# tachyon-beep/shogidrl

Measured on NVIDIA B200. Metric: legal-masked Shogi env steps/sec, higher is better.
Workload: dtype u8

## Files before the change

### shogidrl_b200/csrc/kz_engine.cu

```cuda
#include <cuda_runtime.h>
#include <stddef.h>
#include <stdint.h>
#include "../../include/keisei_b200.h"
#include "kz_common.cuh"

namespace {

__device__ uint32_t g_ray[81 * 8 * 3];
__device__ uint32_t g_step[NCLS * 81 * 3];
__device__ uint32_t g_init_bitmap[BITMAP_WORDS];

__constant__ uint8_t c_init_board[96];
__constant__ uint32_t c_init_key_w;

struct __align__(16) WarpScratch {
  uint32_t bitmap[BITMAP_WORDS];
  uint8_t board[96];
  uint8_t meta[32];
  uint8_t pind[2][96];
  uint32_t pinl[2][8 * 3];
  uint8_t plist[2][40];
  uint8_t dropv[96];
  uint32_t oimg[72];
  float opv[20];
  uint32_t onz;
  uint32_t pad_[3];
};

__shared__ uint32_t s_ray[81 * 8 * 3];
__shared__ uint32_t s_step[NCLS * 81 * 3];
extern __shared__ __align__(16) unsigned char s_dyn[];
#define s_ws (reinterpret_cast<WarpScratch*>(s_dyn))

struct Tables {};

#ifndef KZ_FILL_UNROLL
#define KZ_FILL_UNROLL 1
#endif
#ifndef KZ_FILL_AFTER_COMPACT
#define KZ_FILL_AFTER_COMPACT 1
#endif
#ifndef KZ_ST256
#define KZ_ST256 3
#endif
#ifndef KZ_ROWS_ONCE
#define KZ_ROWS_ONCE 1
#endif
#ifndef KZ_BULK_ZERO
#define KZ_BULK_ZERO 0
#endif
constexpr int kFillUnroll = KZ_FILL_UNROLL;

#if KZ_BULK_ZERO
constexpr int kZeroPage = 16384;
__shared__ __align__(128) unsigned char s_zero[kZeroPage];
__device__ __forceinline__ void bulk_zero(void* dst, uint32_t bytes) {
  const uint32_t src = (uint32_t)__cvta_generic_to_shared(s_zero);
  asm volatile("cp.async.bulk.global.shared::cta.bulk_group [%0], [%1], %2;" ::"l"(dst), "r"(src), "r"(bytes) : "memory");
}
#endif

__device__ __forceinline__ void st_zero256(void* p) {
  const uint32_t z = 0;
  asm volatile("st.global.v8.b32 [%0], {%1,%1,%1,%1,%1,%1,%1,%1};" ::"l"(p), "r"(z) : "memory");
}

__device__ __forceinline__ void st256(void* p, const uint32_t (&v)[8]) {
  asm volatile("st.global.v8.b32 [%0], {%1,%2,%3,%4,%5,%6,%7,%8};" ::"l"(p), "r"(v[0]), "r"(v[1]), "r"(v[2]), "r"(v[3]),
               "r"(v[4]), "r"(v[5]), "r"(v[6]), "r"(v[7]) : "memory");
}

__device__ __forceinline__ BB ld_ray(const Tables&, int sq, int d) {
  const uint32_t* p = s_ray + (sq * 8 + d) * 3;
  return BB{p[0], p[1], p[2]};
}
__device__ __forceinline__ BB ld_step(const Tables&, int cls, int sq) {
  const uint32_t* p = s_step + (cls * 81 + sq) * 3;
  return BB{p[0], p[1], p[2]};
}

__device__ __forceinline__ BB slide_ray(const Tables& T, int sq, int d, BB occ) {
  BB ray = ld_ray(T, sq, d);
  BB bl = ray & occ;
  if (bb_any(bl)) {
    if (dir_positive(d)) ray = ray & bb_upto(bb_lsb(bl));
    else ray = bb_andn(ray, bb_below(bb_msb(bl)));
  }
  return ray;
}

#ifndef KD_ATTR
#define KD_ATTR __forceinline__
#endif
__device__ KD_ATTR BB king_danger(const uint32_t tab, const int K, const int me, const BB occk) {
  const int lane = threadIdx.x & 31;
  const WarpScratch& ws = s_ws[threadIdx.x >> 5];
  const Tables T{};
  const int fwd = me == 0 ? -1 : 1;
  const BB kingsteps = ld_step(T, CLS_KING, K);
// ... 376 lines not shown
  k.z = fmix32(id * 0xC2B2AE3Du + 0x27D4EB2Fu);
  k.w = fmix32(id * 0x27D4EB2Fu + 0x9E3779B9u);
  return k;
}
__device__ __forceinline__ uint4 position_key(const WarpScratch& ws, int lane, int side) {
  uint4 k = make_uint4(0, 0, 0, 0);
#pragma unroll
  for (int j = 0; j < 3; j++) {
    const int sq = lane + 32 * j;
    const int code = sq < 81 ? ws.board[sq] : 0;
    if (code) { uint4 t = zkey_item(sq * 32 + code); k.x ^= t.x; k.y ^= t.y; k.z ^= t.z; k.w ^= t.w; }
  }
  if (lane < 14) {
    const int cnt = ws.meta[lane];
    if (cnt) { uint4 t = zkey_item(4096 + lane * 256 + cnt); k.x ^= t.x; k.y ^= t.y; k.z ^= t.z; k.w ^= t.w; }
  }
  if (lane == 31 && side) { uint4 t = zkey_item(8191); k.x ^= t.x; k.y ^= t.y; k.z ^= t.z; k.w ^= t.w; }
  k.x = __reduce_xor_sync(FULL, k.x);
  k.y = __reduce_xor_sync(FULL, k.y);
  k.z = __reduce_xor_sync(FULL, k.z);
  k.w = __reduce_xor_sync(FULL, k.w);
  return k;
}

struct StepParams {
  uint8_t* boards;
  uint8_t* meta;
  uint4* hist;
  int rep_slots;
  int hist_cap;
  int n;
  int g_first;
  const void* actions;
  int actions_i64;
  float* obs;
  long long obs_stride;
  uint8_t* mask;
  long long mask_stride;
  int mask_vec;
  float* reward;
  uint8_t* done;
  uint8_t* reason;
  int8_t* winner;
  int32_t* ep_len;
  int32_t* legal_count;
  uint8_t* in_check;
  void* next_actions;
  unsigned long long seed;
  uint32_t rng_step;
  uint32_t env_offset;
  int auto_reset;
  int mode;
  int eval_term;
  int* tile_counter;
  uint32_t* bitmap_out;
  long long bitmap_stride;
  uint32_t* cobs_out;
  const uint32_t* pool;
  int pool_size;
  const int32_t* pool_pick;
  unsigned long long pool_seed;
  int32_t* start_ids;
};

__device__ __forceinline__ uint16_t ld_u16(const uint8_t* p) { return (uint16_t)(p[0] | (p[1] << 8)); }
__device__ __forceinline__ void st_u16(uint8_t* p, int v) { p[0] = (uint8_t)v; p[1] = (uint8_t)(v >> 8); }

template <int MODE, bool POOL = false>
__global__ void __launch_bounds__(WARPS_PER_CTA * 32, MIN_CTAS_PER_SM) kz_step_kernel(const StepParams P) {
  for (int i = threadIdx.x; i < 81 * 8 * 3; i += blockDim.x) s_ray[i] = g_ray[i];
  for (int i = threadIdx.x; i < NCLS * 81 * 3; i += blockDim.x) s_step[i] = g_step[i];
#if KZ_BULK_ZERO
  for (int i = threadIdx.x; i < kZeroPage / 16; i += blockDim.x) reinterpret_cast<uint4*>(s_zero)[i] = make_uint4(0, 0, 0, 0);
  asm volatile("fence.proxy.async.shared::cta;" ::: "memory");
#endif
  __syncthreads();
  const Tables T{};
  const int lane = threadIdx.x & 31, warp = threadIdx.x >> 5;
  WarpScratch& ws = s_ws[warp];
  const uint32_t tab = code_info(lane);
  const int g_end = P.g_first + P.n;

  auto fetch_state = [&](int g) -> uint32_t {
    if (g >= g_end) return 0u;
    const uint8_t* src = lane < 24 ? P.boards + (size_t)g * 96 + 4 * lane : P.meta + (size_t)g * 32 + 4 * (lane - 24);
    return *reinterpret_cast<const uint32_t*>(src);
  };
  auto fetch_action = [&](int g) -> long long {
    if (g >= g_end || MODE == 0) return 0;
    return P.actions_i64 ? reinterpret_cast<const long long*>(P.actions)[g]
                         : (long long)reinterpret_cast<const int*>(P.actions)[g];
  };
  const bool lockstep = (P.n % WARPS_PER_CTA) == 0 && P.tile_counter != nullptr;
  const int ntiles = P.n / WARPS_PER_CTA;
  __shared__ int s_tile[4];
  int tile = blockIdx.x, pending = 0;
  if (lockstep && threadIdx.x == 0) {
    s_tile[1] = gridDim.x + atomicAdd(P.tile_counter, 1);
    pending = gridDim.x + atomicAdd(P.tile_counter, 1);
  }
  const int g_stride = gridDim.x * WARPS_PER_CTA;
  int g = P.g_first + blockIdx.x * WARPS_PER_CTA + warp;
  uint32_t next_word = fetch_state(g);
  long long next_action = fetch_action(g);
  __syncthreads();

  for (int it = 0; lockstep ? tile < ntiles : g < g_end; it++) {
    int g_next = g + g_stride;
    if (lockstep) {
      __syncthreads();
      tile = s_tile[(it + 1) & 3];
      g_next = P.g_first + tile * WARPS_PER_CTA + warp;
      if (threadIdx.x == 0) s_tile[(it + 2) & 3] = pending;
    }
    __syncwarp();
    static_assert(offsetof(WarpScratch, meta) == offsetof(WarpScratch, board) + 96, "meta must follow board: one store for all 32 lanes");
    reinterpret_cast<uint32_t*>(ws.board)[lane] = next_word;
    const long long a = next_action;
    next_word = fetch_state(g_next);
    next_action = fetch_action(g_next);
    __syncwarp();
    int side = ws.meta[14];
    int status = ws.meta[15];
    int winner = ws.meta[16] == 0xFF ? -1 : ws.meta[16];
    int err = ws.meta[17];
    int move_count = ld_u16(ws.meta + 18);
    int hist_len = ld_u16(ws.meta + 20);
    const int max_moves = ld_u16(ws.meta + 22);
    uint32_t episodes = ws.meta[24] | (ws.meta[25] << 8) | (ws.meta[26] << 16) | (ws.meta[27] << 24);



    float reward = 0.f;
    int done_out = 0, reason_out = 0, winner_out = -1, ep_len_out = 0;
    bool fresh_senn = false;
    int mover = 1 - side;
    bool moved = false;
    uint4 key = make_uint4(reinterpret_cast<const uint32_t*>(ws.board)[21], reinterpret_cast<const uint32_t*>(ws.board)[22],
                           reinterpret_cast<const uint32_t*>(ws.board)[23], reinterpret_cast<const uint32_t*>(ws.meta)[7]);
    uint32_t kid = 0;
    bool probe = false;
    uint4 probe_e = make_uint4(0, 0, 0, 0);

    if (MODE != 0) {
      if (status != 0) {
      } else if (a < 0 || a >= KZ_NUM_ACTIONS) {
        err |= KZ_ERR_BAD_ACTION;
      } else {
        mover = side;
        const int ai = (int)a;
        bool ok = true;
        if (ai < 12960) {
          const int promo = ai & 1, pair = ai >> 1;
          const int from = pair / 80, t80 = pair - from * 80, to = t80 + (t80 >= from);
          const int code = ws.board[from], tcode = ws.board[to];
          const uint32_t inf = __shfl_sync(FULL, tab, code);
          if (!code || code_color(code) != side) { err |= KZ_ERR_BAD_ACTION; ok = false; }
          else {
            const int fr = sq_row(from), fc = from - 9 * fr, tr = sq_row(to), tc = to - 9 * tr;
            const int dr = tr - fr, dc = tc - fc;
            bool pat;
            if (code_type(code) == 2) {
              pat = dr == (side == 0 ? -2 : 2) && (dc == 1 || dc == -1);
            } else {
              int d = -1;
              if (dc == 0) d = dr < 0 ? 0 : 4;
// ... 68 lines not shown
            key.w ^= __reduce_xor_sync(FULL, dk.w);
          }
          if (hist_len < P.hist_cap) {
            probe = true;
            probe_e = (P.hist + (size_t)g * P.rep_slots)[(key.y + lane) & ((uint32_t)P.rep_slots - 1u)];
            hist_len += 1;
          } else {
            err |= KZ_ERR_HISTORY_FULL;
          }
        }
      }
    }

    auto fill_mask_zero = [&]() {
      if (!P.mask || !P.mask_vec) return;
      uint8_t* mrow = P.mask + (size_t)g * P.mask_stride;
#if (KZ_ST256 & 1)
      if ((((uintptr_t)mrow) & 31) == 0) {
#pragma unroll kFillUnroll
        for (int q = lane; q < 405; q += 32) st_zero256(mrow + 32 * q);
        return;
      }
#endif
      uint4* m4 = reinterpret_cast<uint4*>(mrow);
      const uint4 z4 = make_uint4(0, 0, 0, 0);
#pragma unroll kFillUnroll
      for (int q = lane; q < 810; q += 32) m4[q] = z4;
    };
    auto fill_obs_zero = [&]() {
      if (!P.obs) return;
      float* orow = P.obs + (size_t)g * P.obs_stride;
#if (KZ_ST256 & 2)
      float2* o2 = reinterpret_cast<float2*>(orow);
      const int head = (int)(((32u - (unsigned)((uintptr_t)orow & 31)) & 31u) >> 3);
      const int nb = (KZ_OBS_FLOATS * 4 - head * 8) >> 5;
      char* body = reinterpret_cast<char*>(orow) + head * 8;
      if (lane < head) o2[lane] = make_float2(0.f, 0.f);
#pragma unroll kFillUnroll
      for (int q = lane; q < nb; q += 32) st_zero256(body + 32 * q);
      const int tail0 = head + 4 * nb;
      if (lane < KZ_OBS_FLOATS / 2 - tail0) o2[tail0 + lane] = make_float2(0.f, 0.f);
#else
      const int mis = ((uintptr_t)orow & 15) ? 2 : 0;
      float4* o4 = reinterpret_cast<float4*>(orow + mis);
      const float4 zf = make_float4(0.f, 0.f, 0.f, 0.f);
#pragma unroll kFillUnroll
      for (int q = lane; q < 931; q += 32) o4[q] = zf;
      if (lane == 0) {
        float2* o2 = reinterpret_cast<float2*>(orow + (mis ? 0 : 3724));
        *o2 = make_float2(0.f, 0.f);
      }
#endif
    };
    auto build_obs_image = [&]() {
      __syncwarp();
      ws.oimg[lane] = 0; ws.oimg[lane + 32] = 0;
      if (lane < 8) ws.oimg[lane + 64] = 0;
      float pv = 0.f;
      if (lane < 14) {
        const int cnt = ws.meta[lane < 7 ? side * 7 + lane : (1 - side) * 7 + (lane - 7)];
        if (cnt > 0) pv = __fdiv_rn((float)cnt, 18.0f);
      } else if (lane == 14) pv = side == 0 ? 1.f : 0.f;
      else if (lane == 15) pv = max_moves > 0 ? __fdiv_rn((float)move_count, (float)max_moves) : 0.f;
      if (lane < 20) ws.opv[lane] = pv;
      const uint32_t nz = __ballot_sync(FULL, pv != 0.f);
      if (lane == 0) ws.onz = nz;
      __syncwarp();
#pragma unroll
      for (int j = 0; j < 3; j++) {
        const int sq = lane + 32 * j;
        const int code = sq < 81 ? ws.board[sq] : 0;
        if (code) {
          const int t = code_type(code), mine = code_color(code) == side;
          const int plane = t < 8 ? (mine ? 0 : 14) + t : (mine ? 8 : 22) + (t - 8);
          const int f = plane * 81 + (side == 0 ? sq : 80 - sq);
          atomicOr(&ws.oimg[f >> 5], 1u << (f & 31));
        }
      }
      __syncwarp();
    };
    auto write_obs = [&]() {
      if (!P.obs) return;
      float* orow = P.obs + (size_t)g * P.obs_stride;
#if (KZ_ROWS_ONCE & 2)
      {
        build_obs_image();
        float2* o2 = reinterpret_cast<float2*>(orow);
        const int head = (int)(((32u - (unsigned)((uintptr_t)orow & 31)) & 31u) >> 3);
        const int nb = (KZ_OBS_FLOATS * 4 - head * 8) >> 5;
        char* body = reinterpret_cast<char*>(orow) + head * 8;
        if (lane < head) {
          const uint32_t b2 = ws.oimg[0] >> (2 * lane);
          o2[lane] = make_float2((b2 & 1) ? 1.0f : 0.f, (b2 & 2) ? 1.0f : 0.f);
        }
#pragma unroll 1
        for (int q = lane; q < nb; q += 32) {
          const int r0 = 2 * head + 8 * q;
          char* dst = body + 32 * q;
          if (r0 + 8 <= 28 * 81) {
            const uint32_t bits = __funnelshift_r(ws.oimg[r0 >> 5], ws.oimg[(r0 >> 5) + 1], r0 & 31) & 0xFFu;
            if (bits == 0) st_zero256(dst);
            else {
              uint32_t v[8];
#pragma unroll
              for (int k = 0; k < 8; k++) v[k] = ((bits >> k) & 1) ? 0x3F800000u : 0u;
              st256(dst, v);
            }
          } else {
            const int x = r0 - 28 * 81;
            const int pl0 = x >= 0 ? (x * 1619) >> 17 : -1;
            const int nb0 = (pl0 + 1) * 81 - x;
            const uint32_t a = pl0 >= 0 ? __float_as_uint(ws.opv[pl0]) : 0u, b = __float_as_uint(ws.opv[pl0 + 1]);
            uint32_t bits = 0;
            if (pl0 < 0) bits = __funnelshift_r(ws.oimg[r0 >> 5], ws.oimg[(r0 >> 5) + 1], r0 & 31) & ((1u << nb0) - 1u);
            if (a == 0 && bits == 0 && (nb0 >= 8 || b == 0)) st_zero256(dst);
            else {
              uint32_t v[8];
#pragma unroll
              for (int k = 0; k < 8; k++) v[k] = k < nb0 ? (pl0 >= 0 ? a : (((bits >> k) & 1) ? 0x3F800000u : 0u)) : b;
              st256(dst, v);
            }
          }
        }
        const int tail0 = head + 4 * nb;
        if (lane < KZ_OBS_FLOATS / 2 - tail0) o2[tail0 + lane] = make_float2(0.f, 0.f);
        return;
      }
#endif
      float pv = 0.f;
      if (lane < 14) {
        const int cnt = ws.meta[lane < 7 ? side * 7 + lane : (1 - side) * 7 + (lane - 7)];
        if (cnt > 0) pv = __fdiv_rn((float)cnt, 18.0f);
      } else if (lane == 14) pv = side == 0 ? 1.f : 0.f;
      else if (lane == 15) pv = max_moves > 0 ? __fdiv_rn((float)move_count, (float)max_moves) : 0.f;
      fill_obs_zero();
      __syncwarp();
      uint32_t nzp = __ballot_sync(FULL, pv != 0.f);
      while (nzp) {
        const int i = __ffs(nzp) - 1;
        nzp &= nzp - 1;
        const float v = __shfl_sync(FULL, pv, i);
        float* pl = orow + (28 + i) * 81;
        pl[lane] = v;
        pl[lane + 32] = v;
        if (lane < 17) pl[lane + 64] = v;
      }
#pragma unroll
      for (int j = 0; j < 3; j++) {
        const int sq = lane + 32 * j;
        const int code = sq < 81 ? ws.board[sq] : 0;
        if (code) {
          const int t = code_type(code), mine = code_color(code) == side;
          const int plane = t < 8 ? (mine ? 0 : 14) + t : (mine ? 8 : 22) + (t - 8);
          orow[plane * 81 + (side == 0 ? sq : 80 - sq)] = 1.0f;
        }
      }
    };
    if (MODE == 0) key = position_key(ws, lane, side);
    GenResult gr;
    if constexpr (MODE != 0) {
      gr = gen_moves_impl<true, UFZ_FAST>(tab, side, UFZ_FAST);
    } else {
      int mode = UFZ_GENERIC;
      if (ws.meta[side * 7] > 0) {
        GenResult opp = gen_moves<false>(tab, 1 - side, UFZ_SKIP);
        if (opp.in_check) mode = UFZ_ALL;
      }
      gr = gen_moves<true>(tab, side, mode);
    }

    if (probe) {
      uint4* tb = P.hist + (size_t)g * P.rep_slots;
      const uint32_t smask = (uint32_t)P.rep_slots - 1u;
      uint32_t start = key.y & smask;
      int count = 0;
      uint4 e = probe_e;
      for (int round = 0; round * 32 < P.rep_slots; round++) {
        const uint32_t slot = (start + lane) & smask;
        if (round > 0) e = tb[slot];
        const bool occupied = (e.w & 15u) != 0;
        const bool match = occupied && e.x == key.x && e.y == key.y && e.z == key.z && ((e.w ^ key.w) >> 4) == 0;
        const uint32_t stop = __ballot_sync(FULL, match || !occupied);
        if (stop) {
          const int f = __ffs(stop) - 1;
          const uint32_t oldw = __shfl_sync(FULL, e.w, f);
          const bool was_match = (__ballot_sync(FULL, match) >> f) & 1;
          count = was_match ? min(15, (int)(oldw & 15u) + 1) : 1;
// ... 167 lines not shown
            const uint32_t parts[2] = {v.x, v.y};
            for (int b = 0; b < 7; b++) mrow[13520 + b] = (uint8_t)(parts[b >> 2] >> (8 * (b & 3)));
          }
        }
      } else {
        for (int i = lane; i < KZ_NUM_ACTIONS; i += 32) mrow[i] = (uint8_t)((ws.bitmap[i >> 5] >> (i & 31)) & 1);
      }
    };
    auto pick_next = [&]() {
      if (!P.next_actions) return;
      long long pick = -1;
      if (gr.count > 0) {
        const uint32_t r = rand32(P.seed, (unsigned long long)P.env_offset + (unsigned long long)g, P.rng_step);
        const int k = (int)(((unsigned long long)r * (unsigned long long)gr.count) >> 32);
        const int w0 = lane * 14;
        int pcs[14];
        int mycnt = 0;
#pragma unroll
        for (int i = 0; i < 14; i++) { pcs[i] = __popc(ws.bitmap[w0 + i]); mycnt += pcs[i]; }
        int incl = mycnt;
#pragma unroll
        for (int o = 1; o < 32; o <<= 1) { const int t = __shfl_up_sync(FULL, incl, o); if (lane >= o) incl += t; }
        const int excl = incl - mycnt;
        int found = -1;
        if (k >= excl && k < incl) {
          int rem = k - excl, widx = 0;
          bool open_ = true;
#pragma unroll
          for (int i = 0; i < 14; i++) {
            if (open_) {
              if (rem < pcs[i]) { widx = i; open_ = false; }
              else rem -= pcs[i];
            }
          }
          uint32_t wv = ws.bitmap[w0 + widx];
          for (int r = rem; r > 0; r--) wv &= wv - 1;
          found = (w0 + widx) * 32 + __ffs(wv) - 1;
        }
        const uint32_t who = __ballot_sync(FULL, found >= 0);
        pick = __shfl_sync(FULL, found, __ffs(who) - 1);
      }
      if (lane == 0) {
        if (P.actions_i64) reinterpret_cast<long long*>(P.next_actions)[g] = pick;
        else reinterpret_cast<int*>(P.next_actions)[g] = (int)pick;
      }
    };
    if (MODE == 2 || P.bitmap_out) {
      __syncwarp();
      uint4* dst = reinterpret_cast<uint4*>(P.bitmap_out + (size_t)g * P.bitmap_stride);
      for (int i = lane; i < BITMAP_WORDS / 4; i += 32) dst[i] = reinterpret_cast<const uint4*>(ws.bitmap)[i];
    }
    if constexpr (MODE != 2) write_mask();
    pick_next();
    write_obs();
    if (P.cobs_out) {
      __syncwarp();
      uint8_t* cb = reinterpret_cast<uint8_t*>(ws.oimg);
      if (lane < 21) ws.oimg[lane] = 0xFFFFFFFFu;
      float pv = 0.f;
      if (lane < 14) {
        const int cnt = ws.meta[lane < 7 ? side * 7 + lane : (1 - side) * 7 + (lane - 7)];
        if (cnt > 0) pv = __fdiv_rn((float)cnt, 18.0f);
      } else if (lane == 14) pv = side == 0 ? 1.f : 0.f;
      else if (lane == 15) pv = max_moves > 0 ? __fdiv_rn((float)move_count, (float)max_moves) : 0.f;
      if (lane < 19) ws.oimg[21 + lane] = lane < 18 ? __float_as_uint(pv) : 0u;
      __syncwarp();
#pragma unroll
      for (int j = 0; j < 3; j++) {
        const int sq = lane + 32 * j;
        const int code = sq < 81 ? ws.board[sq] : 0;
        if (code) {
          const int t = code_type(code), mine = code_color(code) == side;
          cb[side == 0 ? sq : 80 - sq] = (uint8_t)(t < 8 ? (mine ? 0 : 14) + t : (mine ? 8 : 22) + (t - 8));
        }
      }
      __syncwarp();
      uint32_t* dst = P.cobs_out + (size_t)g * KZ_COBS_WORDS;
      for (int i = lane; i < KZ_COBS_WORDS; i += 32) dst[i] = ws.oimg[i];
      __syncwarp();
    }

    __syncwarp();
    if (lane == 0) {
      ws.meta[14] = (uint8_t)side;
      ws.meta[15] = (uint8_t)status;
      ws.meta[16] = (uint8_t)(winner < 0 ? 0xFF : winner);
      ws.meta[17] = (uint8_t)err;
      st_u16(ws.meta + 18, move_count);
      st_u16(ws.meta + 20, hist_len);
      ws.meta[24] = (uint8_t)episodes; ws.meta[25] = (uint8_t)(episodes >> 8);
      ws.meta[26] = (uint8_t)(episodes >> 16); ws.meta[27] = (uint8_t)(episodes >> 24);
      reinterpret_cast<uint32_t*>(ws.board)[21] = key.x;
      reinterpret_cast<uint32_t*>(ws.board)[22] = key.y;
      reinterpret_cast<uint32_t*>(ws.board)[23] = key.z;
      reinterpret_cast<uint32_t*>(ws.meta)[7] = key.w;
    }
    __syncwarp();
    {
      uint32_t* bdst = reinterpret_cast<uint32_t*>(P.boards + (size_t)g * 96);
      uint32_t* mdst = reinterpret_cast<uint32_t*>(P.meta + (size_t)g * 32);
      if (lane < 24) bdst[lane] = reinterpret_cast<uint32_t*>(ws.board)[lane];
      else mdst[lane - 24] = reinterpret_cast<uint32_t*>(ws.meta)[lane - 24];
    }
    __syncwarp();
    if (lockstep && threadIdx.x == 0) pending = gridDim.x + atomicAdd(P.tile_counter, 1);
    g = g_next;
  }
#if KZ_BULK_ZERO
  asm volatile("cp.async.bulk.commit_group;" ::: "memory");
  asm volatile("cp.async.bulk.wait_group 0;" ::: "memory");
#endif
}

#ifndef KZ_EXPAND_CTAS_PER_SM
#define KZ_EXPAND_CTAS_PER_SM 1
#endif
#ifndef KZ_EXPAND_PRELOAD
#define KZ_EXPAND_PRELOAD 0
#endif
#ifndef KZ_EXPAND_SPARSE
#define KZ_EXPAND_SPARSE 0
#endif
#ifndef KZ_COMPACT_CTAS_PER_SM
#define KZ_COMPACT_CTAS_PER_SM 2
#endif
__global__ void __launch_bounds__(256) kz_expand_kernel(const uint8_t* __restrict__ boards, const uint8_t* __restrict__ meta,
                                                        const uint32_t* __restrict__ bitmap, int n, float* obs,
                                                        long long obs_stride, uint8_t* mask, long long mask_stride,
                                                        int mask_vec) {
  const int lane = threadIdx.x & 31, warp = threadIdx.x >> 5;
  auto expand = [](uint32_t b16) {
    uint4 v;
    v.x = ((b16 & 0xF) * 0x00204081u) & 0x01010101u;
    v.y = (((b16 >> 4) & 0xF) * 0x00204081u) & 0x01010101u;
    v.z = (((b16 >> 8) & 0xF) * 0x00204081u) & 0x01010101u;
    v.w = (((b16 >> 12) & 0xF) * 0x00204081u) & 0x01010101u;
    return v;
  };
  for (int g = blockIdx.x * 8 + warp; g < n; g += gridDim.x * 8) {
    const uint32_t* bm = bitmap + (size_t)g * BITMAP_WORDS;
    if (mask) {
      uint8_t* mrow = mask + (size_t)g * mask_stride;
      if (mask_vec) {
        uint4* m4 = reinterpret_cast<uint4*>(mrow);
#if KZ_EXPAND_SPARSE
        if (mask_stride >= 13536 && (((uintptr_t)mrow) & 31) == 0) {
          uint32_t wreg[27];
#pragma unroll
          for (int k = 0; k < 27; k++) wreg[k] = lane + 32 * k < 846 ? __ldg(bm + ((lane + 32 * k) >> 1)) : 0u;
#pragma unroll 1
          for (int q = lane; q < 423; q += 32) st_zero256(mrow + 32 * q);
          __syncwarp();
#pragma unroll
          for (int k = 0; k < 27; k++) {
            const int q = lane + 32 * k;
            const uint32_t half = (q & 1) ? (wreg[k] >> 16) : (wreg[k] & 0xFFFF);
            if (q < 846 && half) m4[q] = expand(half);
          }
        } else
#endif
        {
#if KZ_EXPAND_PRELOAD
        uint32_t wreg[27];
#pragma unroll
// ... 221 lines not shown
  if (g >= n) return;
  const Tables T{};
  const uint8_t* b = boards + (size_t)g * 96;
  const int sq = squares[g];
  const uint32_t tab = code_info(lane);
  const int code = (sq >= 0 && sq < 81) ? b[sq] : 0;
  const uint32_t inf = __shfl_sync(FULL, tab, code);
  const int me = code_color(code);
  uint32_t o[3], w[3];
#pragma unroll
  for (int j = 0; j < 3; j++) {
    const int s = lane + 32 * j;
    const int c = s < 81 ? b[s] : 0;
    o[j] = __ballot_sync(FULL, c != 0);
    w[j] = __ballot_sync(FULL, c != 0 && code_color(c) == me);
  }
  BB t = BB{0, 0, 0};
  if (code) {
    t = ld_step(T, (inf >> 16) & 15, sq);
    uint32_t sl = (inf >> 8) & 0xFF;
    while (sl) { const int d = __ffs(sl) - 1; sl &= sl - 1; t = t | slide_ray(T, sq, d, BB{o[0], o[1], o[2]}); }
    t = bb_andn(t, BB{w[0], w[1], w[2]});
  }
  if (lane == 0) { out[(size_t)g * 3] = t.w0; out[(size_t)g * 3 + 1] = t.w1; out[(size_t)g * 3 + 2] = t.w2; }
}

thread_local char t_cuda_err[256] = "";
int cuda_fail(cudaError_t e) {
  snprintf(t_cuda_err, sizeof t_cuda_err, "%s", cudaGetErrorString(e));
  return KZ_E_CUDA;
}
}
int kz_cuda_fail(cudaError_t e) { return cuda_fail(e); }
namespace {
#define CK(x) do { cudaError_t _e = (x); if (_e != cudaSuccess) return cuda_fail(_e); } while (0)

constexpr int kMaxDevices = 64;
int g_sm_counts[kMaxDevices] = {0};
bool g_ready[kMaxDevices] = {false};
inline int cur_device() { int d = 0; return cudaGetDevice(&d) == cudaSuccess && d >= 0 && d < kMaxDevices ? d : -1; }
inline bool host_ready() { const int d = cur_device(); return d >= 0 && g_ready[d]; }
inline int sm_count() { const int d = cur_device(); return d >= 0 ? g_sm_counts[d] : 0; }

struct Layout { int64_t off_boards, off_meta, off_hist, off_sched, total; int rep_slots; };
Layout layout(int n, int hist_cap) {
  Layout L;
  L.rep_slots = 64;
  while (L.rep_slots < 2 * hist_cap) L.rep_slots *= 2;
  L.off_boards = 0;
  L.off_meta = (int64_t)n * 96;
  L.off_hist = L.off_meta + (int64_t)n * 32;
  L.off_hist = (L.off_hist + 255) & ~(int64_t)255;
  L.off_sched = L.off_hist + (int64_t)n * L.rep_slots * 16;
  L.total = L.off_sched + 256;
  return L;
}

int launch_step(void* state, int n, int hist_cap, StepParams P, cudaStream_t st, int first = 0, int count = -1, int slot = 0) {
  if (!state || n <= 0 || hist_cap < 0 || hist_cap > 65535) return KZ_E_ARG;
  if (count < 0) count = n - first;
  if (first < 0 || count <= 0 || first + count > n || slot < 0 || slot >= 64) return KZ_E_ARG;
  if (!host_ready()) return KZ_E_NOT_INIT;
  if (((uintptr_t)state & 255) != 0) return KZ_E_ARG;
  const Layout L = layout(n, hist_cap);
  uint8_t* base = reinterpret_cast<uint8_t*>(state);
  P.boards = base + L.off_boards;
  P.meta = base + L.off_meta;
  P.hist = reinterpret_cast<uint4*>(base + L.off_hist);
  P.rep_slots = L.rep_slots;
  P.hist_cap = hist_cap;
  P.n = count;
  P.g_first = first;
  if (P.obs) {
    if (((uintptr_t)P.obs & 15) || (P.obs_stride & 1) || P.obs_stride < KZ_OBS_FLOATS) return KZ_E_ARG;
  }
  if (P.bitmap_out) {
    if (((uintptr_t)P.bitmap_out & 15) || P.bitmap_stride < BITMAP_WORDS || (P.bitmap_stride & 3)) return KZ_E_ARG;
  } else if (P.mode == 2) return KZ_E_ARG;
  if (P.cobs_out && ((uintptr_t)P.cobs_out & 3)) return KZ_E_ARG;
  P.mask_vec = 0;
  if (P.mask) {
    if (P.mask_stride < KZ_NUM_ACTIONS) return KZ_E_ARG;
    P.mask_vec = (((uintptr_t)P.mask & 15) == 0 && (P.mask_stride & 15) == 0) ? 1 : 0;
    if (count == 1 && ((uintptr_t)P.mask & 15) == 0) P.mask_vec = 1;
  }
  const int ctas_needed = (count + WARPS_PER_CTA - 1) / WARPS_PER_CTA;
  int grid = sm_count() * ((P.mode == 2 && !P.obs) ? KZ_COMPACT_CTAS_PER_SM : CTAS_PER_SM);
  if (grid > ctas_needed) grid = ctas_needed;
  const size_t dyn = sizeof(WarpScratch) * WARPS_PER_CTA;
  P.tile_counter = nullptr;
#ifndef KZ_STATIC_TILES
  if (grid < ctas_needed && count % WARPS_PER_CTA == 0) {
    P.tile_counter = reinterpret_cast<int*>(base + L.off_sched) + slot;
    CK(cudaMemsetAsync(P.tile_counter, 0, sizeof(int), st));
  }
#endif
  if (P.pool) {
    if (P.mode == 1) kz_step_kernel<1, true><<<grid, WARPS_PER_CTA * 32, dyn, st>>>(P);
    else if (P.mode == 2) kz_step_kernel<2, true><<<grid, WARPS_PER_CTA * 32, dyn, st>>>(P);
    else return KZ_E_ARG;
  } else if (P.mode == 1) kz_step_kernel<1><<<grid, WARPS_PER_CTA * 32, dyn, st>>>(P);
  else if (P.mode == 2) kz_step_kernel<2><<<grid, WARPS_PER_CTA * 32, dyn, st>>>(P);
  else kz_step_kernel<0><<<grid, WARPS_PER_CTA * 32, dyn, st>>>(P);
  CK(cudaGetLastError());
  return KZ_OK;
}

}

extern "C" {

int kz_abi_version(void) { return KZ_ABI_VERSION; }
#ifndef KZ_SRC_SHA
#define KZ_SRC_SHA "unknown"
#endif
const char* kz_build_info(void) { return "src_sha=" KZ_SRC_SHA " built=" __DATE__ " " __TIME__ " arch=sm_100a"; }
const char* kz_last_cuda_error(void) { return t_cuda_err; }

int kz_state_layout(int n, int hist_cap, int64_t* offsets3, int64_t* total_bytes) {
  if (n <= 0 || hist_cap < 0 || hist_cap > 65535) return KZ_E_ARG;
  const Layout L = layout(n, hist_cap);
  if (offsets3) { offsets3[0] = L.off_boards; offsets3[1] = L.off_meta; offsets3[2] = L.off_hist; }
  if (total_bytes) *total_bytes = L.total;
  return KZ_OK;
}

int kz_init_tables(void* stream) {
  cudaStream_t st = reinterpret_cast<cudaStream_t>(stream);
  static const int DR[8] = {-1, -1, 0, 1, 1, 1, 0, -1};
  static const int DC[8] = {0, 1, 1, 1, 0, -1, -1, -1};
  static uint32_t ray[81 * 8 * 3];
  static uint32_t step[NCLS * 81 * 3];
  memset(ray, 0, sizeof ray);
  memset(step, 0, sizeof step);
  auto setb = [](uint32_t* bb, int s) { bb[s >> 5] |= 1u << (s & 31); };
  for (int s = 0; s < 81; s++) {
    const int r = s / 9, c = s % 9;
    for (int d = 0; d < 8; d++)
      for (int k = 1; k < 9; k++) {
        const int rr = r + DR[d] * k, cc = c + DC[d] * k;
        if (rr < 0 || rr > 8 || cc < 0 || cc > 8) break;
        setb(ray + (s * 8 + d) * 3, rr * 9 + cc);
      }
    const uint32_t P_ = 0x01, S_ = 0x01 | 0x02 | 0x80 | 0x08 | 0x20, G_ = 0x01 | 0x02 | 0x80 | 0x04 | 0x40 | 0x10;
    const uint32_t PLUS_ = 0x55, X_ = 0xAA, K_ = 0xFF;
    auto rot = [](uint32_t m) { return ((m << 4) | (m >> 4)) & 0xFF; };
    const uint32_t dirsets[NCLS] = {P_, S_, G_, 0, rot(P_), rot(S_), rot(G_), 0, PLUS_, X_, K_, 0};
    for (int cls = 0; cls < NCLS; cls++) {
      uint32_t* bb = step + (cls * 81 + s) * 3;
      for (int d = 0; d < 8; d++)
        if ((dirsets[cls] >> d) & 1) {
          const int rr = r + DR[d], cc = c + DC[d];
          if (rr >= 0 && rr <= 8 && cc >= 0 && cc <= 8) setb(bb, rr * 9 + cc);
        }
      if (cls == CLS_BN || cls == CLS_WN) {
        const int f = cls == CLS_BN ? -1 : 1;
        for (int dc = -1; dc <= 1; dc += 2) {
// ... 27 lines not shown
        k[2] ^= fmix(id * 0xC2B2AE3Du + 0x27D4EB2Fu);
        k[3] ^= fmix(id * 0x27D4EB2Fu + 0x9E3779B9u);
      }
    memcpy(init + 84, k, 12);
    CK(cudaMemcpyToSymbolAsync(c_init_key_w, &k[3], sizeof(uint32_t), 0, cudaMemcpyHostToDevice, st));
  }
  CK(cudaMemcpyToSymbolAsync(c_init_board, init, sizeof init, 0, cudaMemcpyHostToDevice, st));
  int dev = 0;
  CK(cudaGetDevice(&dev));
  if (dev < 0 || dev >= kMaxDevices) return KZ_E_ARG;
  CK(cudaDeviceGetAttribute(&g_sm_counts[dev], cudaDevAttrMultiProcessorCount, dev));
  {
    const int dyn = (int)(sizeof(WarpScratch) * WARPS_PER_CTA);
    CK(cudaFuncSetAttribute(kz_step_kernel<0>, cudaFuncAttributeMaxDynamicSharedMemorySize, dyn));
    CK(cudaFuncSetAttribute(kz_step_kernel<1>, cudaFuncAttributeMaxDynamicSharedMemorySize, dyn));
    CK(cudaFuncSetAttribute(kz_step_kernel<2>, cudaFuncAttributeMaxDynamicSharedMemorySize, dyn));
    CK(cudaFuncSetAttribute(kz_step_kernel<1, true>, cudaFuncAttributeMaxDynamicSharedMemorySize, dyn));
    CK(cudaFuncSetAttribute(kz_step_kernel<2, true>, cudaFuncAttributeMaxDynamicSharedMemorySize, dyn));
  }
  g_ready[dev] = true;
  {
    const Layout L = layout(1, 0);
    void* scratch = nullptr;
    CK(cudaMalloc(&scratch, L.total + KZ_MASK_PAD_STRIDE));
    uint8_t* sb = reinterpret_cast<uint8_t*>(scratch);
    kz_reset_kernel<<<1, 32, 0, st>>>(sb + L.off_boards, sb + L.off_meta, nullptr, 0, 1, nullptr, 500);
    StepParams P{};
    P.mask = sb + L.total;
    P.mask_stride = KZ_MASK_PAD_STRIDE;
    P.mode = 0;
    int rc = launch_step(scratch, 1, 0, P, st);
    if (rc != KZ_OK) { cudaFree(scratch); return rc; }
    CK(cudaStreamSynchronize(st));
    static uint8_t hm[KZ_MASK_PAD_STRIDE];
    CK(cudaMemcpy(hm, sb + L.total, KZ_MASK_PAD_STRIDE, cudaMemcpyDeviceToHost));
    static uint32_t bm[BITMAP_WORDS];
    memset(bm, 0, sizeof bm);
    for (int i = 0; i < KZ_NUM_ACTIONS; i++)
      if (hm[i]) bm[i >> 5] |= 1u << (i & 31);
    CK(cudaMemcpyToSymbol(g_init_bitmap, bm, sizeof bm));
    CK(cudaFree(scratch));
  }
  return KZ_OK;
}

int kz_reset(void* state, int n, int hist_cap, const uint8_t* env_mask, int max_moves, void* stream) {
  if (!state || n <= 0 || max_moves < 0 || max_moves > 65535) return KZ_E_ARG;
  if (!host_ready()) return KZ_E_NOT_INIT;
  const Layout L = layout(n, hist_cap);
  uint8_t* base = reinterpret_cast<uint8_t*>(state);
  kz_reset_kernel<<<(n + 7) / 8, 256, 0, reinterpret_cast<cudaStream_t>(stream)>>>(
      base + L.off_boards, base + L.off_meta, reinterpret_cast<uint4*>(base + L.off_hist), L.rep_slots, n, env_mask, max_moves);
  CK(cudaGetLastError());
  return KZ_OK;
}

int kz_reset_pool(void* state, int n, int hist_cap, const uint8_t* env_mask, int max_moves, const uint32_t* pool, int pool_size,
                  const int32_t* pick, uint64_t pool_seed, uint32_t env_offset, int32_t* start_ids, void* stream) {
  if (!state || n <= 0 || max_moves < 0 || max_moves > 65535 || !pool || pool_size <= 0 || ((uintptr_t)pool & 15))
    return KZ_E_ARG;
  if (!host_ready()) return KZ_E_NOT_INIT;
  const Layout L = layout(n, hist_cap);
  uint8_t* base = reinterpret_cast<uint8_t*>(state);
  kz_reset_pool_kernel<<<(n + 7) / 8, 256, 0, reinterpret_cast<cudaStream_t>(stream)>>>(
      base + L.off_boards, base + L.off_meta, reinterpret_cast<uint4*>(base + L.off_hist), L.rep_slots, n, env_mask, max_moves,
      pool, pool_size, pick, pool_seed, env_offset, start_ids);
  CK(cudaGetLastError());
  return KZ_OK;
}

int kz_pool_records(const void* state, int n, int hist_cap, const uint32_t* bitmap, int64_t bitmap_stride_words,
                    const int32_t* legal_count, const uint8_t* in_check, uint32_t* records, void* stream) {
  if (!state || n <= 0 || hist_cap < 0 || hist_cap > 65535 || !bitmap || bitmap_stride_words < BITMAP_WORDS || !legal_count ||
      !in_check || !records || ((uintptr_t)records & 15))
    return KZ_E_ARG;
  const Layout L = layout(n, hist_cap);
  const uint8_t* base = reinterpret_cast<const uint8_t*>(state);
  kz_pool_records_kernel<<<(n + 7) / 8, 256, 0, reinterpret_cast<cudaStream_t>(stream)>>>(
      base + L.off_boards, base + L.off_meta, n, bitmap, bitmap_stride_words, legal_count, in_check, records);
  CK(cudaGetLastError());
  return KZ_OK;
}

int kz_load_positions(void* state, int n, int hist_cap, const int8_t* boards, const uint8_t* hands,
                      const uint8_t* side, const int32_t* move_count, const int32_t* max_moves, void* stream) {
  if (!state || n <= 0 || !boards || !hands || !side || !move_count || !max_moves) return KZ_E_ARG;
  const Layout L = layout(n, hist_cap);
  uint8_t* base = reinterpret_cast<uint8_t*>(state);
  kz_load_kernel<<<(n + 7) / 8, 256, 0, reinterpret_cast<cudaStream_t>(stream)>>>(
      base + L.off_boards, base + L.off_meta, reinterpret_cast<uint4*>(base + L.off_hist), L.rep_slots, n, boards, hands, side,
      move_count, max_moves);
  CK(cudaGetLastError());
  return KZ_OK;
}

int kz_export_positions(const void* state, int n, int hist_cap, int8_t* boards, uint8_t* hands, int32_t* meta8,
                        void* stream) {
  if (!state || n <= 0) return KZ_E_ARG;
  const Layout L = layout(n, hist_cap);
  const uint8_t* base = reinterpret_cast<const uint8_t*>(state);
  kz_export_kernel<<<(n + 7) / 8, 256, 0, reinterpret_cast<cudaStream_t>(stream)>>>(base + L.off_boards, base + L.off_meta, n,
                                                                                    boards, hands, meta8);
  CK(cudaGetLastError());
  return KZ_OK;
}

int kz_piece_targets(const void* state, int n, int hist_cap, const int32_t* squares, uint32_t* targets3, void* stream) {
  if (!state || n <= 0 || !squares || !targets3) return KZ_E_ARG;
  if (!host_ready()) return KZ_E_NOT_INIT;
  const Layout L = layout(n, hist_cap);
  const uint8_t* base = reinterpret_cast<const uint8_t*>(state);
  kz_targets_kernel<<<(n + 7) / 8, 256, 0, reinterpret_cast<cudaStream_t>(stream)>>>(base + L.off_boards, n, squares, targets3);
  CK(cudaGetLastError());
  return KZ_OK;
}

int kz_errors(void* state, int n, int hist_cap, int32_t* out, int clear, void* stream) {
  if (!state || n <= 0 || !out) return KZ_E_ARG;
  const Layout L = layout(n, hist_cap);
  uint8_t* base = reinterpret_cast<uint8_t*>(state);
  kz_errors_kernel<<<(n + 255) / 256, 256, 0, reinterpret_cast<cudaStream_t>(stream)>>>(base + L.off_meta, n, out, clear);
  CK(cudaGetLastError());
  return KZ_OK;
}

int kz_refresh(void* state, int n, int hist_cap, float* obs, int64_t obs_stride, uint8_t* mask, int64_t mask_stride,
               int32_t* legal_count, void* next_actions, int actions_i64, uint64_t seed, uint32_t rng_step,
               uint32_t env_offset, int eval_termination, uint8_t* in_check, void* stream) {
  StepParams P{};
  P.in_check = in_check;
  P.obs = obs; P.obs_stride = obs_stride; P.mask = mask; P.mask_stride = mask_stride;
  P.legal_count = legal_count; P.next_actions = next_actions; P.actions_i64 = actions_i64;
  P.seed = seed; P.rng_step = rng_step; P.env_offset = env_offset;
  P.mode = 0; P.eval_term = eval_termination;
  return launch_step(state, n, hist_cap, P, reinterpret_cast<cudaStream_t>(stream));
}

int kz_step(void* state, int n, int hist_cap, const void* actions, int actions_i64, float* obs, int64_t obs_stride,
            uint8_t* mask, int64_t mask_stride, float* reward, uint8_t* done, uint8_t* reason, int8_t* winner,
            int32_t* ep_len, int32_t* legal_count, void* next_actions, uint64_t seed, uint32_t rng_step,
            uint32_t env_offset, int auto_reset, void* stream) {
  if (!actions) return KZ_E_ARG;
  StepParams P{};
  P.actions = actions; P.actions_i64 = actions_i64;
  P.obs = obs; P.obs_stride = obs_stride; P.mask = mask; P.mask_stride = mask_stride;
// ... 129 lines not shown
```

Before: 188.9 million.

## Use PDL launches, self-resetting tile counter, vectorized table staging, sparse obs writes

Launches the step kernel with programmatic dependent launch so the next step's table staging can overlap the previous kernel's tail. The per-step cudaMemsetAsync of the tile counter goes away: the last CTA now resets a 64-bit counter that packs completion counts into its high word. Shared tables are loaded as uint4 into registers before griddepcontrol.wait. The observation image is now built with a per-chunk nonzero mask so zero and one-hot stores are split without funnel shifts. This adds complexity and depends on correct PDL and counter-reset ordering across consecutive kernels.

```diff
diff --git a/profiles/step_boundary_probe.py b/profiles/step_boundary_probe.py
--- /dev/null
+++ b/profiles/step_boundary_probe.py
@@ -0,0 +1,114 @@
+from __future__ import annotations
+
+import argparse
+import json
+import os
+import statistics
+import subprocess
+import sys
+import tempfile
+
+import torch
+
+ROOT = os.path.dirname(os.path.dirname(os.path.abspath(__file__)))
+sys.path.insert(0, ROOT)
+
+N, MAX_MOVES, SEED, PREROLL, STEPS = 65536, 500, 2024, 640, 64
+
+
+def main():
+    ap = argparse.ArgumentParser()
+    ap.add_argument("--trace-dir", default=None, help="also keep the chrome traces here")
+    args = ap.parse_args()
+    from torch.profiler import ProfilerActivity, profile
+    from shogidrl_b200 import MASK_PAD_STRIDE, VecShogiEnv, _native
+
+    dev = torch.device("cuda:0")
+    env = VecShogiEnv(N, MAX_MOVES, dev, seed=SEED, auto_reset=True)
+    obs = torch.zeros((2, N, 46, 9, 9), dtype=torch.float32, device=dev)
+    mask = torch.zeros((2, N, MASK_PAD_STRIDE), dtype=torch.uint8, device=dev)
+    act = [torch.zeros(N, dtype=torch.int64, device=dev) for _ in range(2)]
+    it = [0]
+
+    def step():
+        i = it[0]
+        it[0] += 1
+        env.step(act[i & 1], obs=obs[i & 1], mask=mask[i & 1][:, :13527], random_actions=True, next_out=act[(i + 1) & 1])
+
+    env.refresh(random_actions=True, next_out=act[0])
+    for _ in range(PREROLL):
+        step()
+    torch.cuda.synchronize()
+
+    def loop_events():
+        kev = [(torch.cuda.Event(enable_timing=True), torch.cuda.Event(enable_timing=True)) for _ in range(STEPS)]
+        e0, e1 = torch.cuda.Event(enable_timing=True), torch.cuda.Event(enable_timing=True)
+        e0.record()
+        for k in range(STEPS):
+            kev[k][0].record()
+            step()
+            kev[k][1].record()
+        e1.record()
+        torch.cuda.synchronize()
+        return e0.elapsed_time(e1) / STEPS, sum(a.elapsed_time(b) for a, b in kev) / STEPS
+
+    def loop_plain():
+        e0, e1 = torch.cuda.Event(enable_timing=True), torch.cuda.Event(enable_timing=True)
+        e0.record()
+        for _ in range(STEPS):
+            step()
+        e1.record()
+        torch.cuda.synchronize()
+        return e0.elapsed_time(e1) / STEPS
+
+    s = torch.cuda.Stream(dev)
+    s.wait_stream(torch.cuda.current_stream(dev))
+    g = torch.cuda.CUDAGraph()
+    with torch.cuda.graph(g, stream=s):
+        for _ in range(8):
+            step()
+    torch.cuda.current_stream(dev).wait_stream(s)
+    torch.cuda.synchronize()
+
+    def loop_graph():
+        e0, e1 = torch.cuda.Event(enable_timing=True), torch.cuda.Event(enable_timing=True)
+        e0.record()
+        for _ in range(STEPS // 8):
+            g.replay()
+        e1.record()
+        torch.cuda.synchronize()
+        return e0.elapsed_time(e1) / STEPS
+
+    loop_events(); loop_plain(); loop_graph()
+    res = {"events_ms": [], "events_kernel_ms": [], "plain_ms": [], "graph_ms": []}
+    for _ in range(4):
+        a, b = loop_events()
+        res["events_ms"].append(a)
+        res["events_kernel_ms"].append(b)
+        res["plain_ms"].append(loop_plain())
+        res["graph_ms"].append(loop_graph())
+
+    def gaps(fn, name):
+        with profile(activities=[ProfilerActivity.CUDA]) as prof:
+            fn()
+        path = os.path.join(args.trace_dir or tempfile.mkdtemp(), f"step_boundary_{name}.pt.trace.json")
+        prof.export_chrome_trace(path)
+        with open(path) as f:
+            ev = [e for e in json.load(f)["traceEvents"] if e.get("cat") == "kernel" and "kz_step_kernel" in e.get("name", "")]
+        ev.sort(key=lambda e: e["ts"])
+        dur = [e["dur"] for e in ev]
+        gap = [ev[i + 1]["ts"] - (ev[i]["ts"] + ev[i]["dur"]) for i in range(len(ev) - 1)]
+        return {"kernels": len(ev), "dur_us_median": statistics.median(dur), "gap_us_median": statistics.median(gap),
+                "gap_us_min": min(gap), "gap_us_max": max(gap)}
+
+    res["trace_events"] = gaps(loop_events, "events")
+    res["trace_plain"] = gaps(loop_plain, "plain")
+    smi = subprocess.run(["nvidia-smi", "--query-gpu=name,power.limit,clocks.max.sm", "--format=csv,noheader"],
+                         capture_output=True, text=True).stdout.strip()
+    res["gpu"] = smi
+    res["build"] = _native.lib().kz_build_info().decode()
+    print(json.dumps(res))
+
+
+if __name__ == "__main__":
+    main()
diff --git a/shogidrl_b200/csrc/kz_engine.cu b/shogidrl_b200/csrc/kz_engine.cu
--- a/shogidrl_b200/csrc/kz_engine.cu
+++ b/shogidrl_b200/csrc/kz_engine.cu
@@ -6,8 +6,8 @@
 
 namespace {
 
-__device__ uint32_t g_ray[81 * 8 * 3];
-__device__ uint32_t g_step[NCLS * 81 * 3];
+__device__ __align__(16) uint32_t g_ray[81 * 8 * 3];
+__device__ __align__(16) uint32_t g_step[NCLS * 81 * 3];
 __device__ uint32_t g_init_bitmap[BITMAP_WORDS];
 
 __constant__ uint8_t c_init_board[96];
@@ -22,13 +22,12 @@
   uint8_t plist[2][40];
   uint8_t dropv[96];
   uint32_t oimg[72];
+  uint32_t opm[32];
   float opv[20];
-  uint32_t onz;
-  uint32_t pad_[3];
 };
 
-__shared__ uint32_t s_ray[81 * 8 * 3];
-__shared__ uint32_t s_step[NCLS * 81 * 3];
+__shared__ __align__(16) uint32_t s_ray[81 * 8 * 3];
+__shared__ __align__(16) uint32_t s_step[NCLS * 81 * 3];
 extern __shared__ __align__(16) unsigned char s_dyn[];
 #define s_ws (reinterpret_cast<WarpScratch*>(s_dyn))
 
@@ -45,6 +44,9 @@
 #endif
 #ifndef KZ_ROWS_ONCE
 #define KZ_ROWS_ONCE 1
+#endif
+#ifndef KZ_PDL
+#define KZ_PDL 1
 #endif
 #ifndef KZ_BULK_ZERO
 #define KZ_BULK_ZERO 0
@@ -527,7 +529,7 @@
   int auto_reset;
   int mode;
   int eval_term;
-  int* tile_counter;
+  unsigned long long* tile_counter;
   uint32_t* bitmap_out;
   long long bitmap_stride;
   uint32_t* cobs_out;
@@ -543,13 +545,20 @@
 
 template <int MODE, bool POOL = false>
 __global__ void __launch_bounds__(WARPS_PER_CTA * 32, MIN_CTAS_PER_SM) kz_step_kernel(const StepParams P) {
-  for (int i = threadIdx.x; i < 81 * 8 * 3; i += blockDim.x) s_ray[i] = g_ray[i];
-  for (int i = threadIdx.x; i < NCLS * 81 * 3; i += blockDim.x) s_step[i] = g_step[i];
+  constexpr int kRayVec = 81 * 8 * 3 / 4, kTabVec = kRayVec + NCLS * 81 * 3 / 4, kTabPer = (kTabVec + 255) / 256;
+  static_assert(WARPS_PER_CTA * 32 == 256 && (81 * 8 * 3) % 4 == 0 && (NCLS * 81 * 3) % 4 == 0, "table staging layout");
+  uint4 tv[kTabPer];
+#pragma unroll
+  for (int k = 0; k < kTabPer; k++) {
+    const int i = threadIdx.x + 256 * k;
+    if (i < kTabVec)
+      tv[k] = i < kRayVec ? reinterpret_cast<const uint4*>(g_ray)[i] : reinterpret_cast<const uint4*>(g_step)[i - kRayVec];
+  }
 #if KZ_BULK_ZERO
   for (int i = threadIdx.x; i < kZeroPage / 16; i += blockDim.x) reinterpret_cast<uint4*>(s_zero)[i] = make_uint4(0, 0, 0, 0);
   asm volatile("fence.proxy.async.shared::cta;" ::: "memory");
 #endif
-  __syncthreads();
+  asm volatile("griddepcontrol.wait;" ::: "memory");
   const Tables T{};
   const int lane = threadIdx.x & 31, warp = threadIdx.x >> 5;
   WarpScratch& ws = s_ws[warp];
@@ -571,13 +580,20 @@
   __shared__ int s_tile[4];
   int tile = blockIdx.x, pending = 0;
   if (lockstep && threadIdx.x == 0) {
-    s_tile[1] = gridDim.x + atomicAdd(P.tile_counter, 1);
-    pending = gridDim.x + atomicAdd(P.tile_counter, 1);
+    const int first = gridDim.x + (int)atomicAdd(P.tile_counter, 2ull);
+    s_tile[1] = first;
+    pending = first + 1;
   }
   const int g_stride = gridDim.x * WARPS_PER_CTA;
   int g = P.g_first + blockIdx.x * WARPS_PER_CTA + warp;
   uint32_t next_word = fetch_state(g);
   long long next_action = fetch_action(g);
+#pragma unroll
+  for (int k = 0; k < kTabPer; k++) {
+    const int i = threadIdx.x + 256 * k;
+    if (i < kRayVec) reinterpret_cast<uint4*>(s_ray)[i] = tv[k];
+    else if (i < kTabVec) reinterpret_cast<uint4*>(s_step)[i - kRayVec] = tv[k];
+  }
   __syncthreads();
 
   for (int it = 0; lockstep ? tile < ntiles : g < g_end; it++) {
@@ -587,6 +603,7 @@
       tile = s_tile[(it + 1) & 3];
       g_next = P.g_first + tile * WARPS_PER_CTA + warp;
       if (threadIdx.x == 0) s_tile[(it + 2) & 3] = pending;
+      if (tile >= ntiles) asm volatile("griddepcontrol.launch_dependents;");
     }
     __syncwarp();
     static_assert(offsetof(WarpScratch, meta) == offsetof(WarpScratch, board) + 96, "meta must follow board: one store for all 32 lanes");
@@ -761,87 +778,91 @@
       }
 #endif
     };
-    auto build_obs_image = [&]() {
-      __syncwarp();
-      ws.oimg[lane] = 0; ws.oimg[lane + 32] = 0;
-      if (lane < 8) ws.oimg[lane + 64] = 0;
+    auto const_plane_value = [&]() {
       float pv = 0.f;
       if (lane < 14) {
         const int cnt = ws.meta[lane < 7 ? side * 7 + lane : (1 - side) * 7 + (lane - 7)];
         if (cnt > 0) pv = __fdiv_rn((float)cnt, 18.0f);
       } else if (lane == 14) pv = side == 0 ? 1.f : 0.f;
       else if (lane == 15) pv = max_moves > 0 ? __fdiv_rn((float)move_count, (float)max_moves) : 0.f;
-      if (lane < 20) ws.opv[lane] = pv;
-      const uint32_t nz = __ballot_sync(FULL, pv != 0.f);
-      if (lane == 0) ws.onz = nz;
-      __syncwarp();
-#pragma unroll
-      for (int j = 0; j < 3; j++) {
-        const int sq = lane + 32 * j;
-        const int code = sq < 81 ? ws.board[sq] : 0;
-        if (code) {
-          const int t = code_type(code), mine = code_color(code) == side;
-          const int plane = t < 8 ? (mine ? 0 : 14) + t : (mine ? 8 : 22) + (t - 8);
-          const int f = plane * 81 + (side == 0 ? sq : 80 - sq);
-          atomicOr(&ws.oimg[f >> 5], 1u << (f & 31));
-        }
-      }
-      __syncwarp();
+      return pv;
     };
-    auto write_obs = [&]() {
+    auto write_obs = [&](const float pv) {
       if (!P.obs) return;
       float* orow = P.obs + (size_t)g * P.obs_stride;
 #if (KZ_ROWS_ONCE & 2)
-      {
-        build_obs_image();
+      if (MODE != 0) {
         float2* o2 = reinterpret_cast<float2*>(orow);
         const int head = (int)(((32u - (unsigned)((uintptr_t)orow & 31)) & 31u) >> 3);
         const int nb = (KZ_OBS_FLOATS * 4 - head * 8) >> 5;
         char* body = reinterpret_cast<char*>(orow) + head * 8;
+        const int qs = (28 * 81 - 2 * head) >> 3, nimg = (28 * 81 - 2 * head) & 7, qc = qs + (nimg != 0);
+        const int sh = 8 - 2 * head;
+        __syncwarp();
+        if (lane < 18) reinterpret_cast<uint4*>(ws.oimg)[lane] = make_uint4(0, 0, 0, 0);
+        else if (lane < 26) reinterpret_cast<uint4*>(ws.opm)[lane - 18] = make_uint4(0, 0, 0, 0);
+        if (lane < 20) ws.opv[lane] = pv;
+        __syncwarp();
+#pragma unroll
+        for (int j = 0; j < 3; j++) {
+          const int sq = lane + 32 * j;
+          const int code = sq < 81 ? ws.board[sq] : 0;
+          if (code) {
+            const int t = code_type(code), mine = code_color(code) == side;
+            const int plane = t < 8 ? (mine ? 0 : 14) + t : (mine ? 8 : 22) + (t - 8);
+            const int b = plane * 81 + (side == 0 ? sq : 80 - sq) + sh;
+            atomicOr(&ws.oimg[b >> 5], 1u << (b & 31));
+            const int q = (b >> 3) - 1;
+            if (q >= 0 && q < qs) atomicOr(&ws.opm[q & 31], 1u << (q >> 5));
+          }
+        }
+        const uint32_t onz = __ballot_sync(FULL, pv != 0.f);
+        __syncwarp();
+        const uint8_t* img = reinterpret_cast<const uint8_t*>(ws.oimg);
+        const uint32_t* pvu = reinterpret_cast<const uint32_t*>(ws.opv);
+        const uint32_t pm = ws.opm[lane];
+#pragma unroll 1
+        for (int q = lane; q < qs; q += 32)
+          if (!((pm >> (q >> 5)) & 1)) st_zero256(body + 32 * q);
+#pragma unroll 1
+        for (uint32_t m = pm; m; m &= m - 1) {
+          const int q = lane + 32 * (__ffs(m) - 1);
+          const uint32_t bits = img[q + 1];
+          uint32_t v[8];
+#pragma unroll
+          for (int k = 0; k < 8; k++) v[k] = ((bits >> k) & 1) ? 0x3F800000u : 0u;
+          st256(body + 32 * q, v);
+        }
+#pragma unroll 1
+        for (int q = qc + lane; q < nb; q += 32) {
+          const int x = 8 * q + 2 * head - 28 * 81;
+          const int pl = (x * 1619) >> 17;
+          if (((onz >> pl) & 3u) == 0) st_zero256(body + 32 * q);
+          else {
+            const int n0 = 81 * (pl + 1) - x;
+            const uint32_t a = pvu[pl], b = pvu[pl + 1];
+            uint32_t v[8];
+#pragma unroll
+            for (int k = 0; k < 8; k++) v[k] = k < n0 ? a : b;
+            st256(body + 32 * q, v);
+          }
+        }
+        if (lane == 31 && nimg) {
+          const uint32_t bits = img[qs + 1], a = pvu[0];
+          uint32_t v[8];
+#pragma unroll
+          for (int k = 0; k < 8; k++) v[k] = k < nimg ? (((bits >> k) & 1) ? 0x3F800000u : 0u) : a;
+          st256(body + 32 * qs, v);
+        }
         if (lane < head) {
-          const uint32_t b2 = ws.oimg[0] >> (2 * lane);
+          const uint32_t b2 = (uint32_t)img[0] >> (sh + 2 * lane);
           o2[lane] = make_float2((b2 & 1) ? 1.0f : 0.f, (b2 & 2) ? 1.0f : 0.f);
-        }
-#pragma unroll 1
-        for (int q = lane; q < nb; q += 32) {
-          const int r0 = 2 * head + 8 * q;
-          char* dst = body + 32 * q;
-          if (r0 + 8 <= 28 * 81) {
-            const uint32_t bits = __funnelshift_r(ws.oimg[r0 >> 5], ws.oimg[(r0 >> 5) + 1], r0 & 31) & 0xFFu;
-            if (bits == 0) st_zero256(dst);
-            else {
-              uint32_t v[8];
-#pragma unroll
-              for (int k = 0; k < 8; k++) v[k] = ((bits >> k) & 1) ? 0x3F800000u : 0u;
-              st256(dst, v);
-            }
-          } else {
-            const int x = r0 - 28 * 81;
-            const int pl0 = x >= 0 ? (x * 1619) >> 17 : -1;
-            const int nb0 = (pl0 + 1) * 81 - x;
-            const uint32_t a = pl0 >= 0 ? __float_as_uint(ws.opv[pl0]) : 0u, b = __float_as_uint(ws.opv[pl0 + 1]);
-            uint32_t bits = 0;
-            if (pl0 < 0) bits = __funnelshift_r(ws.oimg[r0 >> 5], ws.oimg[(r0 >> 5) + 1], r0 & 31) & ((1u << nb0) - 1u);
-            if (a == 0 && bits == 0 && (nb0 >= 8 || b == 0)) st_zero256(dst);
-            else {
-              uint32_t v[8];
-#pragma unroll
-              for (int k = 0; k < 8; k++) v[k] = k < nb0 ? (pl0 >= 0 ? a : (((bits >> k) & 1) ? 0x3F800000u : 0u)) : b;
-              st256(dst, v);
-            }
-          }
         }
         const int tail0 = head + 4 * nb;
         if (lane < KZ_OBS_FLOATS / 2 - tail0) o2[tail0 + lane] = make_float2(0.f, 0.f);
         return;
       }
 #endif
-      float pv = 0.f;
-      if (lane < 14) {
-        const int cnt = ws.meta[lane < 7 ? side * 7 + lane : (1 - side) * 7 + (lane - 7)];
-        if (cnt > 0) pv = __fdiv_rn((float)cnt, 18.0f);
-      } else if (lane == 14) pv = side == 0 ? 1.f : 0.f;
-      else if (lane == 15) pv = max_moves > 0 ? __fdiv_rn((float)move_count, (float)max_moves) : 0.f;
       fill_obs_zero();
       __syncwarp();
       uint32_t nzp = __ballot_sync(FULL, pv != 0.f);
@@ -1115,17 +1136,12 @@
     }
     if constexpr (MODE != 2) write_mask();
     pick_next();
-    write_obs();
+    write_obs(const_plane_value());
     if (P.cobs_out) {
       __syncwarp();
       uint8_t* cb = reinterpret_cast<uint8_t*>(ws.oimg);
       if (lane < 21) ws.oimg[lane] = 0xFFFFFFFFu;
-      float pv = 0.f;
-      if (lane < 14) {
-        const int cnt = ws.meta[lane < 7 ? side * 7 + lane : (1 - side) * 7 + (lane - 7)];
-        if (cnt > 0) pv = __fdiv_rn((float)cnt, 18.0f);
-      } else if (lane == 14) pv = side == 0 ? 1.f : 0.f;
-      else if (lane == 15) pv = max_moves > 0 ? __fdiv_rn((float)move_count, (float)max_moves) : 0.f;
+      const float pv = const_plane_value();
       if (lane < 19) ws.oimg[21 + lane] = lane < 18 ? __float_as_uint(pv) : 0u;
       __syncwarp();
 #pragma unroll
@@ -1166,13 +1182,16 @@
       else mdst[lane - 24] = reinterpret_cast<uint32_t*>(ws.meta)[lane - 24];
     }
     __syncwarp();
-    if (lockstep && threadIdx.x == 0) pending = gridDim.x + atomicAdd(P.tile_counter, 1);
+    if (lockstep && threadIdx.x == 0) pending = gridDim.x + (int)atomicAdd(P.tile_counter, 1ull);
     g = g_next;
   }
 #if KZ_BULK_ZERO
   asm volatile("cp.async.bulk.commit_group;" ::: "memory");
   asm volatile("cp.async.bulk.wait_group 0;" ::: "memory");
 #endif
+  if (P.tile_counter && threadIdx.x == 0) {
+    if ((atomicAdd(P.tile_counter, 1ull << 32) >> 32) == gridDim.x - 1) atomicExch(P.tile_counter, 0ull);
+  }
 }
 
 #ifndef KZ_EXPAND_CTAS_PER_SM
@@ -1500,7 +1519,7 @@
   L.off_hist = L.off_meta + (int64_t)n * 32;
   L.off_hist = (L.off_hist + 255) & ~(int64_t)255;
   L.off_sched = L.off_hist + (int64_t)n * L.rep_slots * 16;
-  L.total = L.off_sched + 256;
+  L.total = L.off_sched + 512;
   return L;
 }
 
@@ -1539,18 +1558,28 @@
   P.tile_counter = nullptr;
 #ifndef KZ_STATIC_TILES
   if (grid < ctas_needed && count % WARPS_PER_CTA == 0) {
-    P.tile_counter = reinterpret_cast<int*>(base + L.off_sched) + slot;
-    CK(cudaMemsetAsync(P.tile_counter, 0, sizeof(int), st));
-  }
-#endif
+    P.tile_counter = reinterpret_cast<unsigned long long*>(base + L.off_sched) + slot;
+  }
+#endif
+  void (*kern)(const StepParams);
   if (P.pool) {
-    if (P.mode == 1) kz_step_kernel<1, true><<<grid, WARPS_PER_CTA * 32, dyn, st>>>(P);
-    else if (P.mode == 2) kz_step_kernel<2, true><<<grid, WARPS_PER_CTA * 32, dyn, st>>>(P);
+    if (P.mode == 1) kern = kz_step_kernel<1, true>;
+    else if (P.mode == 2) kern = kz_step_kernel<2, true>;
     else return KZ_E_ARG;
-  } else if (P.mode == 1) kz_step_kernel<1><<<grid, WARPS_PER_CTA * 32, dyn, st>>>(P);
-  else if (P.mode == 2) kz_step_kernel<2><<<grid, WARPS_PER_CTA * 32, dyn, st>>>(P);
-  else kz_step_kernel<0><<<grid, WARPS_PER_CTA * 32, dyn, st>>>(P);
-  CK(cudaGetLastError());
+  } else if (P.mode == 1) kern = kz_step_kernel<1>;
+  else if (P.mode == 2) kern = kz_step_kernel<2>;
+  else kern = kz_step_kernel<0>;
+  cudaLaunchConfig_t cfg = {};
+  cfg.gridDim = dim3(grid);
+  cfg.blockDim = dim3(WARPS_PER_CTA * 32);
+  cfg.dynamicSmemBytes = dyn;
+  cfg.stream = st;
+  cudaLaunchAttribute attr[1];
+  attr[0].id = cudaLaunchAttributeProgrammaticStreamSerialization;
+  attr[0].val.programmaticStreamSerializationAllowed = 1;
+  cfg.attrs = attr;
+  cfg.numAttrs = KZ_PDL ? 1 : 0;
+  CK(cudaLaunchKernelEx(&cfg, kern, P));
   return KZ_OK;
 }
 
@@ -1684,6 +1713,7 @@
   kz_reset_kernel<<<(n + 7) / 8, 256, 0, reinterpret_cast<cudaStream_t>(stream)>>>(
       base + L.off_boards, base + L.off_meta, reinterpret_cast<uint4*>(base + L.off_hist), L.rep_slots, n, env_mask, max_moves);
   CK(cudaGetLastError());
+  if (!env_mask) CK(cudaMemsetAsync(base + L.off_sched, 0, L.total - L.off_sched, reinterpret_cast<cudaStream_t>(stream)));
   return KZ_OK;
 }
 
@@ -1723,6 +1753,7 @@
       base + L.off_boards, base + L.off_meta, reinterpret_cast<uint4*>(base + L.off_hist), L.rep_slots, n, boards, hands, side,
       move_count, max_moves);
   CK(cudaGetLastError());
+  CK(cudaMemsetAsync(base + L.off_sched, 0, L.total - L.off_sched, reinterpret_cast<cudaStream_t>(stream)));
   return KZ_OK;
 }
 
```

After: 192.2 million, median of 6. 1.7% higher.
